# KTH-RPL/HiMo

Hardware: AMD Instinct MI355X
Metric: lidar_frames_per_sec_120k (higher is better)
Workload: dtype f16x2 (two-term split fp16, x = h + l with exact subnormals, on the matrix cores; float32 accumulate; ~22-bit products); 1 GPU; per-frame pipeline: pillarise 3 sweeps (512x512 grid) -> SeFlow++-style encoder/decoder + GRU head (random-init, self-specified: reference network source absent) -> per-point flow -> ego-motion removal + dt0 + flow2compDis -> comp_dis; points_per_frame=120000, sweeps_per_frame=3, parallelism=frames sharded x1, refined_output=False, batches_in_flight=3, matrix_arithmetic=f16x2, samples_per_backbone_launch=16, collectives=none (single process)

## Files before the change

### himo_amd/csrc/conv_common.h

```cpp
#pragma once
#include "himo_common.h"
#include "bf16x3.h"
#include <math.h>

namespace himo {

typedef float floatx16 __attribute__((ext_vector_type(16)));

enum Epilogue {
    kEpiBias = 0,
    kEpiBiasBnGelu = 1,
    kEpiBiasGelu = 2,
    kEpiGruZR = 3,
    kEpiGruQ = 4,
    kEpiBiasRelu = 5,
    kEpiReluMask = 6
};

struct ConvArgs {
    const float* x; int64_t x_batch_stride; int x_pitch;
    const float* w;
    const float* bias; const float* scale; const float* shift;
    float* y; int64_t y_batch_stride; int y_pitch;
    int N, H, W, Cin, Cout;
    int n_inner; int64_t x_outer_stride, y_outer_stride;
    int Ho, Wo;
    const float* aux_in; int aux_in_pitch;
    float* aux_out; int aux_out_pitch;
    int act_flags;
    unsigned* range_seen;
    const unsigned long long* mask;
    int64_t mask_batch_stride, mask_outer_stride;
};
enum ActFlags { kActSplitIn = 1, kActSplitOut = 2, kActVecStore = 4, kActAccumulate = 8, kActStuffedIn = 16, kActRowMask = 32 };

__device__ inline int64_t image_offset(int img, int n_inner, int64_t batch_stride, int64_t outer_stride) {
    return (int64_t)(img % n_inner) * batch_stride + (int64_t)(img / n_inner) * outer_stride;
}

__device__ inline int xcd_block_id(int bid, int n_blocks) {
    const int per = n_blocks >> 3, rem = n_blocks & 7;
    const int xcd = bid & 7, idx = bid >> 3;
    return xcd * per + (xcd < rem ? xcd : rem) + idx;
}

__device__ inline float gelu_exact(float v) {
    const float hv = 0.5f * v;
    const float t = __builtin_amdgcn_rcpf(fmaf(0.3275911f * 0.70710678118654752440f, fabsf(v), 1.0f));
    float p = fmaf(1.061405429f, t, -1.453152027f);
// ... 154 lines not shown
```

### himo_amd/csrc/conv_plan.h

```cpp
#pragma once
#include "conv_common.h"

namespace himo {

enum ConvFamily {
    kConvF32,
    kConvStaged,
    kConvFromL2,
    kConvPresplit3,
    kConvPresplit1
};

struct ConvPlan {
    ConvFamily family;
    ConvArgs args;
    int ks, stride, epi, fmt;
    int bn, mi, ph, nt;
    const void* w_packed;
    dim3 grid;
    const char* prof_name;
};

void launch_conv_f32(const ConvPlan& p, hipStream_t s);
void launch_conv_staged(const ConvPlan& p, hipStream_t s);
// ... 115 lines not shown
    a.H = d.h; a.W = d.w_in; a.Cin = d.cin; a.Cout = d.cout;
    a.Ho = d.stride == 2 ? (d.h + 1) / 2 : d.h;
    a.Wo = d.stride == 2 ? (d.w_in + 1) / 2 : d.w_in;
    a.aux_in = d.aux_in; a.aux_in_pitch = d.aux_in_pitch; a.aux_out = d.aux_out; a.aux_out_pitch = d.aux_out_pitch;
    a.act_flags = d.act_layout;
    a.range_seen = (d.act_layout & kActSplitOut) ? d.d_range_seen : nullptr;

    if (d.act_layout & kActRowMask) {
        if (!d.d_mask || (reinterpret_cast<uintptr_t>(d.d_mask) & 7u)) return HIMO_ERR_INVALID_ARGUMENT;
        if (d.act_layout != (kActRowMask | kActSplitIn) || !d.w_packed || d.packed_format != 1 || d.ksize != 3 || d.stride != 1 ||
            d.cout > 64 || (d.w_in & 31) || (d.epilogue != kEpiBias && d.epilogue != kEpiBiasBnGelu) || (d.cin & 15) || (d.x_pitch & 15))
            return HIMO_ERR_UNSUPPORTED;
        a.mask = reinterpret_cast<const unsigned long long*>(d.d_mask);
        a.mask_batch_stride = d.mask_batch_stride; a.mask_outer_stride = d.mask_outer_stride;
    }
    const bool gemm_acc = d.act_layout == kActAccumulate && d.w_packed && d.ksize == 1 && d.epilogue == kEpiBias && (d.packed_format == 0 || d.packed_format == 2);
    if (d.act_layout & (kActAccumulate | kActStuffedIn)) {
        if (!gemm_acc && ((d.act_layout & ~(kActAccumulate | kActStuffedIn)) || !d.w_packed || d.packed_format != 2 || d.ksize != 3 ||
                          d.stride != 1 || d.epilogue != kEpiBias))
            return HIMO_ERR_UNSUPPORTED;
        if ((d.act_layout & kActStuffedIn) && ((d.h & 1) || (d.w_in & 1) || !below_2gb((int64_t)(d.h / 2) * (d.w_in / 2), d.x_pitch)))
            return HIMO_ERR_UNSUPPORTED;
    } else if (d.act_layout && !(d.act_layout & kActRowMask)) {
        if ((d.act_layout & ~(kActSplitIn | kActSplitOut)) || !d.w_packed || d.packed_format != 1) return HIMO_ERR_UNSUPPORTED;
        if (d.ksize == 1 && !(d.act_layout & kActSplitIn)) return HIMO_ERR_UNSUPPORTED;
        if (d.epilogue != kEpiBias && d.epilogue != kEpiBiasBnGelu) return HIMO_ERR_UNSUPPORTED;
        if (((d.act_layout & kActSplitIn) && ((d.cin & 15) || (d.x_pitch & 15))) ||
            ((d.act_layout & kActSplitOut) && ((d.cout & 15) || (d.y_pitch & 15))))
            return HIMO_ERR_UNSUPPORTED;
    }

    const int hint = d.tile_hint, rows_hint = hint & 15;
    const bool l2_hint = hint == 0 || (hint & 0x1000);
    if (!d.w_packed || (d.stride == 2 && (gru || !l2_hint))) {
        p.family = kConvF32;
        plan_staged_tile(p, 4, 16, d.epilogue == kEpiGruZR, hint);
        p.prof_name = conv_prof_name(d.ksize, d.stride, -1);
        if (d.ksize == 1 && vec_store_ok(a) && !(a.Cout & 31) && (d.epilogue != kEpiReluMask || (aligned16(a.aux_in) && !(a.aux_in_pitch & 3))))
            a.act_flags |= kActVecStore;
// ... 20 lines not shown
```

### himo_amd/csrc/convsg.hip

```cpp
#include "conv_plan.h"
#include "bf16x3.h"
#include <type_traits>

namespace himo {

__device__ __attribute__((aligned(64))) unsigned char g_zero_page[64];


__device__ inline void glds16(const void* gsrc, unsigned lds_dst) {
    unsigned keep;
    asm volatile("s_mov_b32 %0, m0\n\ts_mov_b32 m0, %2\n\ts_nop 0\n\tglobal_load_lds_dwordx4 %1, off\n\ts_mov_b32 m0, %0"
                 : "=&s"(keep) : "v"(gsrc), "s"(lds_dst) : "memory");
}

template <int EPI, int PH, int MI, bool OSPLIT, int S, int NT = 1>
__global__ __launch_bounds__(256, NT == 2 ? (MI == 2 ? 3 : 2) : (S == 2 || MI == 4) ? 3 : 4)
void conv3_presplit_kernel(ConvArgs a, const unsigned short* __restrict__ wpk) {
    constexpr int TW = 32, TH = MI * PH, PHt = S == 1 ? TH + 2 : 2 * TH + 1, PWP = S == 1 ? 40 : 80, UPR = PWP / 16;
    constexpr int kRow = PWP * 64, kBuf = (PHt * kRow + 1023) / 1024 * 1024;
    constexpr int kUnits = S == 1 ? (PHt * PWP + 15) / 16 : PHt * UPR, kUPW = (kUnits + 3) / 4;
    constexpr int BN = (4 / PH) * 32 * NT;
    __shared__ __attribute__((aligned(1024))) unsigned char patch[2 * kBuf];

    const int n_tiles_n = (a.Cout + BN - 1) / BN;
    int bid = xcd_block_id(blockIdx.x, gridDim.x);
    const int tn = bid % n_tiles_n; bid /= n_tiles_n;
    const int tx = (a.Wo + TW - 1) / TW, ty = (a.Ho + TH - 1) / TH;
    const int ox0 = (bid % tx) * TW; bid /= tx;
    const int oy0 = (bid % ty) * TH;
    const int img = bid / ty;
    const unsigned char* __restrict__ xin = reinterpret_cast<const unsigned char*>(a.x + image_offset(img, a.n_inner, a.x_batch_stride, a.x_outer_stride));
    const int slabs = a.Cin >> 4;

    const int wave = __builtin_amdgcn_readfirstlane(threadIdx.x >> 6), lane = threadIdx.x & 63;
    const int wp = wave % PH, wc = wave / PH;
    const int li = lane & 31, lh = lane >> 5;
    const int co = tn * BN + wc * NT * 32 + li;
    const bool co_ok = co < a.Cout;
    const int iy0 = oy0 * S - 1, ix0 = ox0 * S - 1;
    const unsigned lds_base = (unsigned)(uintptr_t)(__attribute__((address_space(3))) unsigned char*)(&patch[0]);

    int src[kUPW];
#pragma unroll
    for (int k = 0; k < kUPW; ++k) {
        const int u = wave + 4 * k;
        const int q = u * 16 + (lane >> 2);
        const int row = S == 1 ? q / PWP : u / UPR, px = S == 1 ? q - row * PWP : (u % UPR) * 16 + (lane >> 2);
        const int col = S == 1 ? px : px < 48 ? 2 * px : 2 * (px - 48) + 1;
        const int iy = iy0 + row, ix = ix0 + col;
        const bool ok = u < kUnits && row < PHt && (S == 1 ? px < TW + 2 : px <= 32 || px >= 48) && iy >= 0 && iy < a.H && ix >= 0 && ix < a.W;
        const int sl = (lane & 3) ^ ((px >> 2) & 3);
        src[k] = ok ? (int)((((int64_t)iy * a.W + ix) * a.x_pitch) * 4 + sl * 16) : -1;
    }
    const unsigned char* zero = g_zero_page + (lane & 3) * 16;
    auto stage = [&](int slab, int buf) {
#pragma unroll
        for (int k = 0; k < kUPW; ++k) {
            const int u = wave + 4 * k;
            if (u < kUnits)
                glds16(src[k] >= 0 ? xin + (unsigned)(src[k] + slab * 64) : zero,
                       lds_base + buf * kBuf + (S == 1 ? u * 1024 : ((u / UPR) * PWP + (u % UPR) * 16) * 64));
        }
    };

    floatx16 acc[MI][NT];
#pragma unroll
    for (int mi = 0; mi < MI; ++mi)
#pragma unroll
        for (int nt = 0; nt < NT; ++nt)
#pragma unroll
            for (int r = 0; r < 16; ++r) acc[mi][nt][r] = 0.f;

    const unsigned char* __restrict__ wb = reinterpret_cast<const unsigned char*>(wpk);
    unsigned b_lane[NT];
#pragma unroll
    for (int nt = 0; nt < NT; ++nt) {
// ... 295 lines not shown
#pragma unroll
                for (int j = 0; j < 4; ++j) {
                    const int pxl = (four >> (8 * j)) & 255;
                    if (e0 + 8 * g + j < n_occ && co < a.Cout)
                        yout[((int64_t)(oy0 + (pxl >> 5)) * a.Wo + (ox0 + (pxl & 31))) * a.y_pitch + co] = epi_activate<EPI>(acc[mi][4 * g + j], eA, eB);
                }
            }
        }
    };
    if (mine_n == 1) { run(std::integral_constant<int, 1>{}); return; }
    if (mine_n == 2) { run(std::integral_constant<int, 2>{}); return; }
    if (mine_n == 3) { run(std::integral_constant<int, 3>{}); return; }
    run(std::integral_constant<int, 4>{});
}

template <int EPI, int PH, int MI, bool OSPLIT>
__global__ __launch_bounds__(256, 4)
void conv1_presplit_kernel(ConvArgs a, const unsigned short* __restrict__ wpk) {
    constexpr int G = 2, TH = MI * PH, BM = TH * 32;
    constexpr int kSeg = 32 * 64, kSlab = TH * kSeg, kBuf = G * kSlab;
    constexpr int kUnits = G * TH * 2, kUPW = (kUnits + 3) / 4;
    constexpr int BN = (4 / PH) * 32;
    __shared__ __attribute__((aligned(1024))) unsigned char patch[2 * kBuf < 16384 ? 16384 : 2 * kBuf];

    const int n_tiles_n = (a.Cout + BN - 1) / BN;
    int bid = xcd_block_id(blockIdx.x, gridDim.x);
    const int tn = bid % n_tiles_n; bid /= n_tiles_n;
    const int64_t rows = (int64_t)a.Ho * a.Wo;
    const int tiles = (int)((rows + BM - 1) / BM);
    const int img = bid / tiles;
    const int64_t row0 = (int64_t)(bid % tiles) * BM;
// ... 4 lines not shown
    const int wp = wave % PH, wc = wave / PH;
    const int li = lane & 31, lh = lane >> 5;
    const int co = tn * BN + wc * 32 + li;
    const bool co_ok = co < a.Cout;
    const unsigned lds_base = (unsigned)(uintptr_t)(__attribute__((address_space(3))) unsigned char*)(&patch[0]);

    int src[kUPW];
#pragma unroll
    for (int k = 0; k < kUPW; ++k) {
        const int u = wave + 4 * k;
        const int g = u / (2 * TH), seg = (u >> 1) % TH, px = (u & 1) * 16 + (lane >> 2);
        const int64_t pix = row0 + seg * 32 + px;
        const int sl = (lane & 3) ^ ((px >> 2) & 3);
        src[k] = (u < kUnits && pix < rows) ? (int)(pix * a.x_pitch * 4 + sl * 16 + g * 64) : -1;
    }
    const unsigned char* zero = g_zero_page + (lane & 3) * 16;
    auto stage = [&](int step, int buf) {
#pragma unroll
        for (int k = 0; k < kUPW; ++k) {
            const int u = wave + 4 * k;
            if (u < kUnits) {
                const int g = u / (2 * TH);
                const bool ok = src[k] >= 0 && step * G + g < slabs;
                glds16(ok ? xin + (unsigned)(src[k] + step * (G * 64)) : zero, lds_base + buf * kBuf + g * kSlab + ((u >> 1) % TH) * kSeg + (u & 1) * 1024);
            }
        }
    };

    floatx16 acc[MI];
#pragma unroll
    for (int mi = 0; mi < MI; ++mi)
#pragma unroll
        for (int r = 0; r < 16; ++r) acc[mi][r] = 0.f;

    const int co_ld = co_ok ? co : a.Cout - 1;
    const unsigned char* __restrict__ wb = reinterpret_cast<const unsigned char*>(wpk);
    const unsigned b_lane = (unsigned)co_ld * 32u + (unsigned)lh * 16u, b_plane = (unsigned)a.Cout * 32u;
    auto load_b = [&](int slab, uint4 (&b)[2]) {
        const unsigned off = (unsigned)slab * (2u * b_plane) + b_lane;
        b[0] = *reinterpret_cast<const uint4*>(wb + off);
// ... 70 lines not shown
                else yout[pix * a.y_pitch + co] = v;
            }
        }
    }
}

#define HIMO_SG(KERNEL, E, O, ...) hipLaunchKernelGGL((KERNEL<E, PH, MI, O, ##__VA_ARGS__>), p.grid, dim3(256), 0, s, p.args, (const unsigned short*)p.w_packed)
#define HIMO_SG_EPI(KERNEL, ...)                                                                                                          \
    do {                                                                                                                                  \
        const bool osplit = (p.args.act_flags & kActSplitOut) != 0;                                                                       \
        if (p.epi == kEpiBias) { if (osplit) HIMO_SG(KERNEL, kEpiBias, true, ##__VA_ARGS__); else HIMO_SG(KERNEL, kEpiBias, false, ##__VA_ARGS__); } \
        else { if (osplit) HIMO_SG(KERNEL, kEpiBiasBnGelu, true, ##__VA_ARGS__); else HIMO_SG(KERNEL, kEpiBiasBnGelu, false, ##__VA_ARGS__); }       \
    } while (0)

template <int PH, int MI>
static void launch_sg1(const ConvPlan& p, hipStream_t s) { HIMO_SG_EPI(conv1_presplit_kernel); }

template <int PH, int MI, int S = 1, int NT = 1>
static void launch_sg(const ConvPlan& p, hipStream_t s) { HIMO_SG_EPI(conv3_presplit_kernel, S, NT); }
#undef HIMO_SG_EPI
#undef HIMO_SG

void launch_conv_presplit1(const ConvPlan& p, hipStream_t s) {
    if (p.ph == 1) {
        if (p.mi == 4) launch_sg1<1, 4>(p, s);
        else if (p.mi == 2) launch_sg1<1, 2>(p, s);
        else launch_sg1<1, 1>(p, s);
    } else {
        if (p.mi == 2) launch_sg1<2, 2>(p, s);
        else launch_sg1<2, 1>(p, s);
    }
}

void launch_conv_presplit3(const ConvPlan& p, hipStream_t s) {
    if (p.args.act_flags & kActRowMask) {
        if (p.epi == kEpiBias) hipLaunchKernelGGL((conv3_rowmask_kernel<kEpiBias>), p.grid, dim3(256), 0, s, p.args, (const unsigned short*)p.w_packed);
        else hipLaunchKernelGGL((conv3_rowmask_kernel<kEpiBiasBnGelu>), p.grid, dim3(256), 0, s, p.args, (const unsigned short*)p.w_packed);
        return;
    }
    if (p.stride == 2) { if (p.ph == 1) launch_sg<1, 2, 2>(p, s); else launch_sg<2, 1, 2>(p, s); }
    else if (p.nt == 2) {
        if (p.ph == 4) launch_sg<4, 2, 1, 2>(p, s);
        else if (p.ph == 1) launch_sg<1, 4, 1, 2>(p, s);
        else launch_sg<2, 4, 1, 2>(p, s);
    }
    else if (p.ph == 1) {
        if (p.mi == 4) launch_sg<1, 4>(p, s);
        else if (p.mi == 2) launch_sg<1, 2>(p, s);
        else launch_sg<1, 1>(p, s);
    } else {
        if (p.mi == 2) launch_sg<2, 2>(p, s);
        else launch_sg<2, 1>(p, s);
    }
}

// ... 2 lines not shown
```

### himo_amd/pipeline.py

```python
from __future__ import annotations

from dataclasses import dataclass

import numpy as np
import torch

from . import _lib
from .compdis import CompDisEngine, FrameBatch
from .seflow.model import SeFlowNet


@dataclass
class Sample:
    pch1: torch.Tensor
    pc0: torch.Tensor
    pc1: torch.Tensor
    pose_h1: np.ndarray
    pose0: np.ndarray
    pose1: np.ndarray
    lidar_dt: torch.Tensor
    scene_id: str = ""
    timestamp: int = 0

    @classmethod
# ... 66 lines not shown
            meta=[(s.scene_id, s.timestamp) for s in samples])
        return self._batch

    def _forward(self, samples, outs) -> None:
        mb = self.net.max_batch
        for lo in range(0, len(samples), mb):
            grp = samples[lo:lo + mb]
            self.net.forward_batch([(s.pch1, s.pc0, s.pc1, s.pose_h1, s.pose0, s.pose1) for s in grp], outs[lo:lo + mb])

    def _set_sparse_dec4(self):
        net = self.net
        if hasattr(net, "sparse_dec4"):
            net.sparse_dec4 = bool(net.precision == "f16x2" and net.fused_head and net.split_acts)
            if hasattr(net, "head_offsets_only"):
                net.head_offsets_only = net.sparse_dec4

    def _fall_back(self):
        self.net = SeFlowNet(precision="bf16x3", **self._net_args)
        self._set_sparse_dec4()

    def _guard_begin(self):
        if self.net.precision == "f16x2":
            if not self.net.fused_head:
                raise RuntimeError("precision='f16x2' needs the fused head: its output stage carries the finite-flow guard")
            self.net.clear_nonfinite()

    def _guard_now(self) -> bool:
        if self.net.precision != "f16x2":
            return True
        self._guard_why = self.net.guard_verdict(self.net.guard.cpu().tolist())
# ... 150 lines not shown
```

### himo_amd/seflow/model.py

```python
from __future__ import annotations

import ctypes

import numpy as np
import torch

from .. import _lib
from . import spec

EPI_BIAS, EPI_BIAS_BN_GELU, EPI_BIAS_GELU, EPI_GRU_ZR, EPI_GRU_Q = range(5)


class ConvDesc(ctypes.Structure):
    _fields_ = [("x", ctypes.c_void_p), ("x_batch_stride", ctypes.c_int64), ("x_pitch", ctypes.c_int),
                ("w", ctypes.c_void_p), ("bias", ctypes.c_void_p), ("scale", ctypes.c_void_p), ("shift", ctypes.c_void_p),
                ("y", ctypes.c_void_p), ("y_batch_stride", ctypes.c_int64), ("y_pitch", ctypes.c_int),
                ("n", ctypes.c_int), ("h", ctypes.c_int), ("w_in", ctypes.c_int), ("cin", ctypes.c_int),
                ("cout", ctypes.c_int), ("ksize", ctypes.c_int), ("stride", ctypes.c_int), ("epilogue", ctypes.c_int),
                ("aux_in", ctypes.c_void_p), ("aux_in_pitch", ctypes.c_int),
                ("aux_out", ctypes.c_void_p), ("aux_out_pitch", ctypes.c_int), ("w_packed", ctypes.c_void_p),
                ("tile_hint", ctypes.c_int), ("packed_format", ctypes.c_int),
                ("n_outer", ctypes.c_int), ("x_outer_stride", ctypes.c_int64), ("y_outer_stride", ctypes.c_int64),
                ("act_layout", ctypes.c_int), ("range_seen", ctypes.c_void_p),
                ("mask", ctypes.c_void_p), ("mask_batch_stride", ctypes.c_int64), ("mask_outer_stride", ctypes.c_int64)]


ACT_SPLIT_IN, ACT_SPLIT_OUT = 1, 2
ACT_ROW_MASK = 32
ACT_ACCUMULATE = 8
ACT_STUFFED_2X = 16
PILLAR_NO_LISTS, PILLAR_HALFWAVE_ONLY = 4, 8


_lib.register({
    "himo_pillar_workspace_bytes": (ctypes.c_size_t, [ctypes.c_int64, ctypes.c_int, ctypes.c_int]),
    "himo_pillar_occupancy_reset": (ctypes.c_int, [ctypes.c_void_p, ctypes.c_size_t, ctypes.c_int, ctypes.c_int, ctypes.c_void_p]),
    "himo_pillarize": (ctypes.c_int, [ctypes.c_int64, ctypes.c_void_p, ctypes.c_int, ctypes.POINTER(ctypes.c_float),
                                      ctypes.POINTER(ctypes.c_float), ctypes.POINTER(ctypes.c_float),
                                      ctypes.POINTER(ctypes.c_float), ctypes.c_int, ctypes.c_int,
                                      ctypes.c_void_p, ctypes.c_void_p, ctypes.c_void_p,
                                      ctypes.c_void_p, ctypes.c_void_p, ctypes.c_void_p, ctypes.c_void_p,
                                      ctypes.c_int, ctypes.c_void_p, ctypes.c_size_t, ctypes.c_void_p]),
    "himo_conv2d": (ctypes.c_int, [ctypes.POINTER(ConvDesc), ctypes.c_void_p]),
# ... 92 lines not shown
            raise ValueError("max_batch")
        self.max_batch = max_batch
        self.precision = precision
        self.autotune = autotune
        self.keep_cell_lists = False
        self.fused_head = precision != "f32"
        self._incremental_images = True
        self.use_plan = True
        self.use_graph = True
        self._plans = {}
        self._recording = None
        self._nb = 1
        self.packed_format = 1 if precision == "f16x2" else 0
        self._split_acts = precision == "f16x2"
        self._sparse_dec4 = False
        self.head_offsets_only = False
        self.tiles = {}
        self.lib = _lib.load()
        self.device = device if device is not None else _lib.require_gpu()
        params = spec.init_params(seed) if params is None else params
        shapes = spec.param_shapes()
        for k, shp in shapes.items():
            if k not in params or tuple(params[k].shape) != tuple(shp):
                raise KeyError(f"parameter {k} missing or of wrong shape (want {shp})")
        cpu = {k: torch.from_numpy(np.ascontiguousarray(params[k], dtype=np.float32)) for k in shapes}
        def fold(prefix, eps):
            scale = cpu[f"{prefix}.gamma"] / torch.sqrt(cpu[f"{prefix}.var"] + eps)
            return scale, cpu[f"{prefix}.beta"] - cpu[f"{prefix}.mean"] * scale
        derived = {}
        derived["pfn.scale"], derived["pfn.shift"] = fold("pfn.bn", spec.BN_EPS_PFN)
# ... 45 lines not shown
        self.F1 = buf((H // 2) * (W // 2), 64 * F)
        self.E2 = [buf(F, (H // 4) * (W // 4), 128) for _ in range(2)]
        self.F2 = buf((H // 4) * (W // 4), 128 * F)
        self.E3 = [buf(F, (H // 8) * (W // 8), 256) for _ in range(2)]
        self.F3 = buf((H // 8) * (W // 8), 256 * F)
        self.T1 = buf((H // 8) * (W // 8), 256)
        self.CAT1 = buf((H // 4) * (W // 4), 512)
        self.S = [buf((H // 4) * (W // 4), 256) for _ in range(2)]
        self.T2 = buf((H // 4) * (W // 4), 128)
        self.CAT2 = buf((H // 2) * (W // 2), 256)
        self.T = [buf((H // 2) * (W // 2), 128) for _ in range(2)]
        self.T3 = buf((H // 2) * (W // 2), 64)
        self.CAT3 = buf(H * W, 128)
        self.U = [buf(H * W, 64) for _ in range(2)]
        self.DEC = buf(H * W, 64)
        self.occ0 = torch.zeros((B, (H * W + 63) // 64), dtype=torch.int64, device=dev)
        self.max_points = 0
        self._reserve_points(max_points)
        self.guard = torch.zeros(2 + self.MAX_RANGE_SLOTS, dtype=torch.int32, device=dev)
        self.nonfinite = self.guard[:1]
        self._ran_word = self.guard[-1:]
        self._range_slots = {}
        self._range = _f32x(spec.POINT_CLOUD_RANGE[:3])
        self._voxel = _f32x(spec.VOXEL_SIZE)
        r, v = spec.POINT_CLOUD_RANGE, spec.VOXEL_SIZE
        self._centre = _f32x([v[0] / 2 + r[0], v[1] / 2 + r[1], v[2] / 2 + r[2]])

    def _reserve_points(self, n: int):
        if n <= self.max_points:
            return
        dev = self.device
# ... 23 lines not shown
        if on != self._incremental_images:
            self._incremental_images = on
            self.reset_images()

    @property
    def split_acts(self) -> bool:
        return self._split_acts

    @split_acts.setter
    def split_acts(self, on: bool):
        on = bool(on)
        if on != self._split_acts:
            self._split_acts = on
            if not on:
                self._sparse_dec4 = False
            self.drop_plan()
            self.reset_images()

    HEAD_SLOT = 1

    @property
    def sparse_dec4(self) -> bool:
        return self._sparse_dec4

    @sparse_dec4.setter
    def sparse_dec4(self, on: bool):
        on = bool(on)
        if on and not (self.packed_format == 1 and self._split_acts and self.fused_head):
            raise ValueError("sparse_dec4 needs precision='f16x2' with split activations and the fused head")
        if on != self._sparse_dec4:
            self._sparse_dec4 = on
            self.drop_plan()

    @property
    def B0(self):
        return self._B0

    @B0.setter
    def B0(self, buf):
        self._B0 = buf
        self.drop_plan()
        self.reset_images()

    MAX_RANGE_SLOTS = 63

    def clear_nonfinite(self):
        _lib.check(self.lib.himo_clear_u32(self.guard.data_ptr(), self.guard.numel(), _lib.stream_handle()), "himo_clear_u32")

    def _range_word(self, wname: str) -> int:
# ... 11 lines not shown
        return None

    def reset_images(self):
        for st in getattr(self, "_pt", ()):
            for ws in st["ws_slots"]:
                _lib.check(self.lib.himo_pillar_occupancy_reset(ws.data_ptr(), ws.numel(), self.W, self.H, _lib.stream_handle()),
                           "himo_pillar_occupancy_reset")

    def _use_sample(self, i: int):
        st = self._pt[i]
        self._sample = i
        self.ws_slots, self.xyz_t, self.pid, self.offsets = st["ws_slots"], st["xyz_t"], st["pid"], st["offsets"]

    def _conv(self, x, x_bs, x_pitch, wname, y, y_bs, y_pitch, n, h, w, cin, cout, ks, stride, epi, x_off=0, y_off=0,
              scale=None, shift=None, aux_in=None, aux_in_pitch=0, aux_out=None, aux_out_pitch=0, bias=None, batched=True,
              act=0, mask=None):
        d = ConvDesc()
        d.x = x.data_ptr() + 4 * x_off; d.x_batch_stride = x_bs; d.x_pitch = x_pitch
        if batched and self._nb > 1:
            d.n_outer, d.x_outer_stride, d.y_outer_stride = self._nb, x.stride(0), y.stride(0)
        d.w = self.p[f"{wname}.weight"].data_ptr()
        d.bias = (self.p[f"{wname}.bias"] if bias is None else bias).data_ptr()
        d.scale = None if scale is None else scale.data_ptr()
        d.shift = None if shift is None else shift.data_ptr()
        d.y = y.data_ptr() + 4 * y_off; d.y_batch_stride = y_bs; d.y_pitch = y_pitch
        d.n, d.h, d.w_in, d.cin, d.cout, d.ksize, d.stride, d.epilogue = n, h, w, cin, cout, ks, stride, epi
        d.aux_in = None if aux_in is None else aux_in.data_ptr(); d.aux_in_pitch = aux_in_pitch
        d.aux_out = None if aux_out is None else aux_out.data_ptr(); d.aux_out_pitch = aux_out_pitch
        pk = self.packed.get(f"{wname}.weight")
        d.w_packed = None if pk is None else pk.data_ptr()
        d.packed_format = self.packed_format
        d.act_layout = act if self.split_acts else 0
        if mask is not None:
            d.act_layout |= ACT_ROW_MASK
            d.mask, d.mask_batch_stride, d.mask_outer_stride = mask.data_ptr(), 0, mask.stride(0)
        if (d.act_layout & ACT_SPLIT_OUT) and self.packed_format == 1 and epi in (EPI_BIAS, EPI_BIAS_BN_GELU):
            d.range_seen = self._range_word(wname)
        key = (n * max(d.n_outer, 1), h, w, cin, cout, ks, stride, epi, pk is not None, d.act_layout)
        if self.autotune and key not in self.tiles:
            self.tiles[key] = self._tune(d)
        d.tile_hint = self.tiles.get(key, 0)
        if self._recording is not None and epi not in (EPI_GRU_ZR, EPI_GRU_Q):
            op = HimoOp(); op.kind = 0; op.conv = d
            self._recording.append(op)
        _lib.check(self.lib.himo_conv2d(ctypes.byref(d), _lib.stream_handle()), f"himo_conv2d({wname})")

    def _tune(self, d: "ConvDesc") -> int:
        if d.epilogue in (EPI_GRU_ZR, EPI_GRU_Q) or (d.act_layout & ACT_ROW_MASK):
            return 0
        cands = [(bn << 4) | mi for bn in (128, 64) if not (bn == 128 and d.cout % 128) for mi in (2, 1)]
# ... 54 lines not shown
    def encoder(self):
        H, W, F = self.H, self.W, self.F
        p = self.p
        stages = [("enc1", 4, 32, 64, H, W, self.E1, self.F1), ("enc2", 6, 64, 128, H // 2, W // 2, self.E2, self.F2),
                  ("enc3", 6, 128, 256, H // 4, W // 4, self.E3, self.F3)]
        src, src_bs, src_pitch = self.B0, 32, 32 * F
        for stage, n_conv, cin, cout, h, w, pingpong, catbuf in stages:
            ho, wo = h // 2, w // 2
            for i in range(n_conv):
                name = f"{stage}.{i}"
                last = i == n_conv - 1
                dst = catbuf if last else pingpong[i % 2]
                dst_bs, dst_pitch = (cout, cout * F) if last else (ho * wo * cout, cout)
                act = ACT_SPLIT_IN | ACT_SPLIT_OUT
                if i == 0:
                    self._conv(src, src_bs, src_pitch, name, dst, dst_bs, dst_pitch, F, h, w, cin, cout, 3, 2,
                               EPI_BIAS_BN_GELU, scale=p[f"{name}.scale"], shift=p[f"{name}.shift"], act=act)
                else:
                    self._conv(src, src_bs, src_pitch, name, dst, dst_bs, dst_pitch, F, ho, wo, cout, cout, 3, 1,
                               EPI_BIAS_BN_GELU, scale=p[f"{name}.scale"], shift=p[f"{name}.shift"], act=act)
                src, src_bs, src_pitch = dst, dst_bs, dst_pitch

    def decoder(self):
        H, W, F = self.H, self.W, self.F
        IN, IO = ACT_SPLIT_IN, ACT_SPLIT_IN | ACT_SPLIT_OUT
        fold = self.fold_decoder
        def block(name, coarse, c_in, ch, cw, tmp, cat, skip, skip_c, lat, out, work, nxt=None):
            if coarse is not None:
                self._conv(coarse, 0, c_in, f"{name}.u1", tmp, 0, lat, 1, 1, ch * cw, c_in, lat, 1, 1, EPI_BIAS, act=IN)
            self._up(tmp, lat, ch, cw, lat, cat, 2 * lat, out_split=True)
            self._conv(skip, 0, skip_c, f"{name}.u3", cat, 0, 2 * lat, 1, 1, 4 * ch * cw, skip_c, lat, 1, 1, EPI_BIAS, y_off=lat, act=IO)
            self._conv(cat, 0, 2 * lat, f"{name}.u4", work[0], 0, out, 1, 2 * ch, 2 * cw, 2 * lat, out, 3, 1, EPI_BIAS, act=IO)
            if fold and nxt is not None:
                nname, ntmp, nlat = nxt
                self._conv(work[0], 0, out, f"{name}.u5>{nname}.u1", ntmp, 0, nlat, 1, 2 * ch, 2 * cw, out, nlat, 3, 1, EPI_BIAS, act=IN)
                return None
            self._conv(work[0], 0, out, f"{name}.u5", work[1], 0, out, 1, 2 * ch, 2 * cw, out, out, 3, 1, EPI_BIAS, act=IO)
            return work[1]
        s = block("dec1", self.F3, 256 * F, H // 8, W // 8, self.T1, self.CAT1, self.F2, 128 * F, 256, 256, self.S, ("dec2", self.T2, 128))
        t = block("dec2", s, 256, H // 4, W // 4, self.T2, self.CAT2, self.F1, 64 * F, 128, 128, self.T, ("dec3", self.T3, 64))
        u = block("dec3", t, 128, H // 2, W // 2, self.T3, self.CAT3, self.B0, 32 * F, 64, 64, self.U)
        self._conv(u, 0, 64, "dec4", self.DEC, 0, 64, 1, H, W, 64, 64, 3, 1, EPI_BIAS, act=IN,
                   mask=self.occ0 if self._sparse_dec4 else None)
        return self.DEC

    def head(self, pc0: torch.Tensor, slot0: int = 1, slot1: int = 2, out: torch.Tensor | None = None) -> torch.Tensor:
# ... 112 lines not shown
        lean = self.head_offsets_only and not self.keep_cell_lists
        for lo in range(0, len(jobs), per_call):
            grp = jobs[lo:lo + per_call]
            arr = (HimoSweep * (len(grp) * self.F))()
            for j, (sample, sweeps, transforms) in enumerate(grp):
                st = self._pt[sample]
                for slot, (pts, T) in enumerate(zip(sweeps, transforms)):
                    w = arr[j * self.F + slot]
                    w.n, w.d_pts, w.pc_stride = pts.shape[0], pts.data_ptr(), pts.shape[1]
                    w.transform = _f32x(np.asarray(T, dtype=np.float32).reshape(-1))
                    w.d_xyz_t, w.d_pid, w.d_offsets = st["xyz_t"][slot].data_ptr(), st["pid"][slot].data_ptr(), st["offsets"][slot].data_ptr()
                    if lean and slot != self.HEAD_SLOT:
                        w.d_offsets = None
                    w.d_image = self.B0[sample].data_ptr() + 4 * 32 * slot
                    w.d_workspace = st["ws_slots"][slot].data_ptr()
                    w.d_occupancy = self.occ0[sample].data_ptr() if slot == self.HEAD_SLOT else None
            status = self.lib.himo_pillarize_multi_ex(len(arr), ctypes.addressof(arr), self._range, self._voxel, self._centre, self.W, self.H,
                                                      self.p["pfn.weight"].data_ptr(), self.p["pfn.scale"].data_ptr(),
                                                      self.p["pfn.shift"].data_ptr(), 32 * self.F, self._pt[0]["ws_slots"][0].numel(),
                                                      (1 if self.split_acts else 0) | (2 if self.incremental_images else 0) |
                                                      (PILLAR_NO_LISTS if lean else 0), _lib.stream_handle())
            _lib.check(status, "himo_pillarize_multi_ex")

    def pillar_features(self, sweeps, transforms, scale: torch.Tensor, shift: torch.Tensor):
        arr = (HimoSweep * self.F)()
        st = self._pt[self._sample]
        for slot, (pts, T) in enumerate(zip(sweeps, transforms)):
            w = arr[slot]
            w.n, w.d_pts, w.pc_stride = pts.shape[0], pts.data_ptr(), pts.shape[1]
            w.transform = _f32x(np.asarray(T, dtype=np.float32).reshape(-1))
            w.d_xyz_t, w.d_pid, w.d_offsets = st["xyz_t"][slot].data_ptr(), st["pid"][slot].data_ptr(), st["offsets"][slot].data_ptr()
# ... 3 lines not shown
                                                     self.p["pfn.weight"].data_ptr(), scale.data_ptr(), shift.data_ptr(), 32 * self.F,
                                                     st["ws_slots"][0].numel(),
                                                     (1 if self.split_acts else 0) | (2 if self.incremental_images else 0), _lib.stream_handle())
        _lib.check(status, "himo_pillar_features_multi")

    def pillarize_into(self, slot: int, pts: torch.Tensor, transform):
        n = pts.shape[0]
        self._reserve_points(n)
        arr = (HimoSweep * 1)()
        w = arr[0]
        w.n, w.d_pts, w.pc_stride = n, pts.data_ptr(), pts.shape[1]
        w.transform = _f32x(np.asarray(transform, dtype=np.float32).reshape(-1))
        w.d_xyz_t, w.d_pid, w.d_offsets = self.xyz_t[slot].data_ptr(), self.pid[slot].data_ptr(), self.offsets[slot].data_ptr()
        w.d_image = self.B0[self._sample].data_ptr() + 4 * 32 * slot
        w.d_workspace = self.ws_slots[slot].data_ptr()
        w.d_occupancy = self.occ0[self._sample].data_ptr() if slot == self.HEAD_SLOT else None
        st = self.lib.himo_pillarize_multi_ex(1, ctypes.addressof(arr), self._range, self._voxel, self._centre, self.W, self.H,
                                              self.p["pfn.weight"].data_ptr(), self.p["pfn.scale"].data_ptr(),
                                              self.p["pfn.shift"].data_ptr(), 32 * self.F, self.ws_slots[slot].numel(),
                                              (1 if self.split_acts else 0) | (2 if self.incremental_images else 0), _lib.stream_handle())
        _lib.check(st, "himo_pillarize_multi_ex")


def conv2d_nhwc(x: torch.Tensor, weight: torch.Tensor, bias: torch.Tensor, stride: int = 1, epilogue: int = EPI_BIAS,
                scale: torch.Tensor | None = None, shift: torch.Tensor | None = None, precision: str = "f32",
                tile_hint: int = 0, act_layout: int = 0, out: torch.Tensor | None = None) -> torch.Tensor:
    lib = _lib.load()
    n, h, w, cin = x.shape
    k, _, _, cout = weight.shape
    stuffed = bool(act_layout & ACT_STUFFED_2X)
    if stuffed:
# ... 32 lines not shown
```

### include/himo_amd.h

```cpp
#ifndef HIMO_AMD_H
#define HIMO_AMD_H

#include <stddef.h>
#include <stdint.h>

#ifdef __cplusplus
extern "C" {
#endif

#define HIMO_ABI_VERSION 1

typedef enum himo_status {
    HIMO_OK = 0,
    HIMO_ERR_INVALID_ARGUMENT = 1,
    HIMO_ERR_EMPTY_FRAME = 2,
    HIMO_ERR_WORKSPACE = 3,
    HIMO_ERR_SINGULAR_POSE = 4,
    HIMO_ERR_HIP = 5,
    HIMO_ERR_UNSUPPORTED = 6
} himo_status;

#define HIMO_FLAG_F32_CHAIN 0x1u
#define HIMO_FLAG_RAW 0x2u
#define HIMO_FLAG_SCANIA 0x4u
// ... 397 lines not shown
    const float* w;
    const float* bias; const float* scale; const float* shift;
    float* y; int64_t y_batch_stride; int y_pitch;
    int n, h, w_in, cin, cout, ksize, stride, epilogue;
    const float* aux_in; int aux_in_pitch;
    float* aux_out; int aux_out_pitch;
    const void* w_packed;
    int tile_hint;
    int packed_format;
    int n_outer;
    int64_t x_outer_stride, y_outer_stride;
    int act_layout;
    uint32_t* d_range_seen;
    const uint64_t* d_mask;
    int64_t mask_batch_stride, mask_outer_stride;
} himo_conv_desc;
#define HIMO_ACT_SPLIT_IN 1
#define HIMO_ACT_SPLIT_OUT 2
#define HIMO_ACT_ROW_MASK 32
#define HIMO_ACT_ACCUMULATE 8
#define HIMO_ACT_STUFFED_2X 16
int himo_conv2d(const himo_conv_desc* h_desc, void* stream);
size_t himo_conv_packed_weight_bytes(int ksize, int cin, int cout);
int himo_conv_pack_weights(const float* d_w, int ksize, int cin, int cout, void* d_packed, void* stream);
#define HIMO_PACK_BF16X3 0
#define HIMO_PACK_F16X2 1
#define HIMO_PACK_BF16X2 2
int himo_conv_pack_weights_ex(const float* d_w, int ksize, int cin, int cout, int format, void* d_packed, void* stream);

int himo_upsample2x(const float* d_x, int x_pitch, int h, int w, int c, float* d_y, int y_pitch, void* stream);
int himo_upsample2x_batch(int n, const float* d_x, int64_t x_batch_stride, int x_pitch, int h, int w, int c, float* d_y,
                          int64_t y_batch_stride, int y_pitch, void* stream);
int himo_upsample2x_batch_ex(int n, const float* d_x, int64_t x_batch_stride, int x_pitch, int h, int w, int c, float* d_y,
                             int64_t y_batch_stride, int y_pitch, int out_split, void* stream);
// ... 279 lines not shown
```

Baseline: 772.6 frames/s.

## Skip loading empty pillars in first encoder and skip convs via occupancy masks

The pillarize step now writes a per-sweep occupancy bitmask for all slots instead of only the head slot. The first stride-2 encoder conv and the decoder's 1x1 skip conv on B0 read these masks and stage zeros from a zero page for unoccupied pixels, per channel group, instead of fetching them from global memory. This cuts global memory traffic on the sparse pillar image. The cost is extra mask reads and bit bookkeeping in the staging loops, plus more template variants.

```diff
diff --git a/himo_amd/csrc/conv_common.h b/himo_amd/csrc/conv_common.h
--- a/himo_amd/csrc/conv_common.h
+++ b/himo_amd/csrc/conv_common.h
@@ -31,8 +31,9 @@
     unsigned* range_seen;
     const unsigned long long* mask;
     int64_t mask_batch_stride, mask_outer_stride;
+    int mask_group_steps; int64_t mask_group_stride;
 };
-enum ActFlags { kActSplitIn = 1, kActSplitOut = 2, kActVecStore = 4, kActAccumulate = 8, kActStuffedIn = 16, kActRowMask = 32 };
+enum ActFlags { kActSplitIn = 1, kActSplitOut = 2, kActVecStore = 4, kActAccumulate = 8, kActStuffedIn = 16, kActRowMask = 32, kActInMask = 64 };
 
 __device__ inline int64_t image_offset(int img, int n_inner, int64_t batch_stride, int64_t outer_stride) {
     return (int64_t)(img % n_inner) * batch_stride + (int64_t)(img / n_inner) * outer_stride;
diff --git a/himo_amd/csrc/conv_plan.h b/himo_amd/csrc/conv_plan.h
--- a/himo_amd/csrc/conv_plan.h
+++ b/himo_amd/csrc/conv_plan.h
@@ -153,6 +153,17 @@
         a.mask = reinterpret_cast<const unsigned long long*>(d.d_mask);
         a.mask_batch_stride = d.mask_batch_stride; a.mask_outer_stride = d.mask_outer_stride;
     }
+    if (d.act_layout & kActInMask) {
+        if (!d.d_mask || (reinterpret_cast<uintptr_t>(d.d_mask) & 7u) || d.mask_group_channels < 0) return HIMO_ERR_INVALID_ARGUMENT;
+        const int gch = d.mask_group_channels ? d.mask_group_channels : d.cin;
+        if ((d.act_layout & ~(kActInMask | kActSplitIn | kActSplitOut)) || !(d.act_layout & kActSplitIn) || !d.w_packed || d.packed_format != 1 ||
+            !(d.ksize == 1 || d.stride == 2) || (d.ksize == 3 && d.tile_hint && !(d.tile_hint & 0x1000)) ||
+            (gch & 31) || d.cin % gch || d.cin / gch > 32)
+            return HIMO_ERR_UNSUPPORTED;
+        a.mask = reinterpret_cast<const unsigned long long*>(d.d_mask);
+        a.mask_batch_stride = d.mask_batch_stride; a.mask_outer_stride = d.mask_outer_stride;
+        a.mask_group_steps = gch / (d.ksize == 1 ? 32 : 16); a.mask_group_stride = d.mask_group_stride;
+    }
     const bool gemm_acc = d.act_layout == kActAccumulate && d.w_packed && d.ksize == 1 && d.epilogue == kEpiBias && (d.packed_format == 0 || d.packed_format == 2);
     if (d.act_layout & (kActAccumulate | kActStuffedIn)) {
         if (!gemm_acc && ((d.act_layout & ~(kActAccumulate | kActStuffedIn)) || !d.w_packed || d.packed_format != 2 || d.ksize != 3 ||
@@ -161,7 +172,7 @@
         if ((d.act_layout & kActStuffedIn) && ((d.h & 1) || (d.w_in & 1) || !below_2gb((int64_t)(d.h / 2) * (d.w_in / 2), d.x_pitch)))
             return HIMO_ERR_UNSUPPORTED;
     } else if (d.act_layout && !(d.act_layout & kActRowMask)) {
-        if ((d.act_layout & ~(kActSplitIn | kActSplitOut)) || !d.w_packed || d.packed_format != 1) return HIMO_ERR_UNSUPPORTED;
+        if ((d.act_layout & ~(kActSplitIn | kActSplitOut | kActInMask)) || !d.w_packed || d.packed_format != 1) return HIMO_ERR_UNSUPPORTED;
         if (d.ksize == 1 && !(d.act_layout & kActSplitIn)) return HIMO_ERR_UNSUPPORTED;
         if (d.epilogue != kEpiBias && d.epilogue != kEpiBiasBnGelu) return HIMO_ERR_UNSUPPORTED;
         if (((d.act_layout & kActSplitIn) && ((d.cin & 15) || (d.x_pitch & 15))) ||
diff --git a/himo_amd/csrc/convsg.hip b/himo_amd/csrc/convsg.hip
--- a/himo_amd/csrc/convsg.hip
+++ b/himo_amd/csrc/convsg.hip
@@ -13,7 +13,7 @@
                  : "=&s"(keep) : "v"(gsrc), "s"(lds_dst) : "memory");
 }
 
-template <int EPI, int PH, int MI, bool OSPLIT, int S, int NT = 1>
+template <int EPI, int PH, int MI, bool OSPLIT, int S, int NT = 1, bool IM = false>
 __global__ __launch_bounds__(256, NT == 2 ? (MI == 2 ? 3 : 2) : (S == 2 || MI == 4) ? 3 : 4)
 void conv3_presplit_kernel(ConvArgs a, const unsigned short* __restrict__ wpk) {
     constexpr int TW = 32, TH = MI * PH, PHt = S == 1 ? TH + 2 : 2 * TH + 1, PWP = S == 1 ? 40 : 80, UPR = PWP / 16;
@@ -41,6 +41,10 @@
     const unsigned lds_base = (unsigned)(uintptr_t)(__attribute__((address_space(3))) unsigned char*)(&patch[0]);
 
     int src[kUPW];
+    unsigned occ[kUPW];
+    int grp_left = IM ? a.mask_group_steps : 0;
+    const unsigned* __restrict__ mw = IM ? reinterpret_cast<const unsigned*>(a.mask + image_offset(img, a.n_inner, a.mask_batch_stride, a.mask_outer_stride)) : nullptr;
+    const int groups = IM ? slabs / a.mask_group_steps : 0;
 #pragma unroll
     for (int k = 0; k < kUPW; ++k) {
         const int u = wave + 4 * k;
@@ -51,6 +55,14 @@
         const bool ok = u < kUnits && row < PHt && (S == 1 ? px < TW + 2 : px <= 32 || px >= 48) && iy >= 0 && iy < a.H && ix >= 0 && ix < a.W;
         const int sl = (lane & 3) ^ ((px >> 2) & 3);
         src[k] = ok ? (int)((((int64_t)iy * a.W + ix) * a.x_pitch) * 4 + sl * 16) : -1;
+        if (IM) {
+            occ[k] = 0u;
+            if (ok) {
+                const int pix = iy * a.W + ix;
+                for (int g = 0; g < groups; ++g)
+                    occ[k] |= ((mw[2 * (g * a.mask_group_stride) + (pix >> 5)] >> (pix & 31)) & 1u) << g;
+            }
+        }
     }
     const unsigned char* zero = g_zero_page + (lane & 3) * 16;
     auto stage = [&](int slab, int buf) {
@@ -58,8 +70,13 @@
         for (int k = 0; k < kUPW; ++k) {
             const int u = wave + 4 * k;
             if (u < kUnits)
-                glds16(src[k] >= 0 ? xin + (unsigned)(src[k] + slab * 64) : zero,
+                glds16((IM ? (occ[k] & 1u) != 0 : src[k] >= 0) ? xin + (unsigned)(src[k] + slab * 64) : zero,
                        lds_base + buf * kBuf + (S == 1 ? u * 1024 : ((u / UPR) * PWP + (u % UPR) * 16) * 64));
+        }
+        if (IM && --grp_left == 0) {
+            grp_left = a.mask_group_steps;
+#pragma unroll
+            for (int k = 0; k < kUPW; ++k) occ[k] >>= 1;
         }
     };
 
@@ -385,7 +402,7 @@
     run(std::integral_constant<int, 4>{});
 }
 
-template <int EPI, int PH, int MI, bool OSPLIT>
+template <int EPI, int PH, int MI, bool OSPLIT, bool IM = false>
 __global__ __launch_bounds__(256, 4)
 void conv1_presplit_kernel(ConvArgs a, const unsigned short* __restrict__ wpk) {
     constexpr int G = 2, TH = MI * PH, BM = TH * 32;
@@ -420,6 +437,28 @@
         const int sl = (lane & 3) ^ ((px >> 2) & 3);
         src[k] = (u < kUnits && pix < rows) ? (int)(pix * a.x_pitch * 4 + sl * 16 + g * 64) : -1;
     }
+    unsigned occ[kUPW];
+    int grp_left = IM ? a.mask_group_steps : 0;
+    if (IM) {
+        const unsigned long long* __restrict__ mw = a.mask + image_offset(img, a.n_inner, a.mask_batch_stride, a.mask_outer_stride);
+        const int groups = steps / a.mask_group_steps;
+#pragma unroll
+        for (int k = 0; k < kUPW; ++k) occ[k] = 0u;
+        for (int g = 0; g < groups; ++g) {
+#pragma unroll
+            for (int k = 0; k < kUPW; ++k) {
+                const int u = wave + 4 * k;
+                const int64_t pix0 = row0 + ((u >> 1) % TH) * 32 + (u & 1) * 16;
+                if (u < kUnits && pix0 < rows) {
+                    const unsigned long long word = mw[g * a.mask_group_stride + (pix0 >> 6)];
+                    occ[k] |= (unsigned)((word >> ((int)(pix0 & 63) + (lane >> 2))) & 1ull) << g;
+                }
+            }
+        }
+#pragma unroll
+        for (int k = 0; k < kUPW; ++k)
+            if (src[k] < 0) occ[k] = 0u;
+    }
     const unsigned char* zero = g_zero_page + (lane & 3) * 16;
     auto stage = [&](int step, int buf) {
 #pragma unroll
@@ -427,9 +466,14 @@
             const int u = wave + 4 * k;
             if (u < kUnits) {
                 const int g = u / (2 * TH);
-                const bool ok = src[k] >= 0 && step * G + g < slabs;
+                const bool ok = (IM ? (occ[k] & 1u) != 0 : src[k] >= 0) && step * G + g < slabs;
                 glds16(ok ? xin + (unsigned)(src[k] + step * (G * 64)) : zero, lds_base + buf * kBuf + g * kSlab + ((u >> 1) % TH) * kSeg + (u & 1) * 1024);
             }
+        }
+        if (IM && --grp_left == 0) {
+            grp_left = a.mask_group_steps;
+#pragma unroll
+            for (int k = 0; k < kUPW; ++k) occ[k] >>= 1;
         }
     };
 
@@ -530,10 +574,13 @@
     } while (0)
 
 template <int PH, int MI>
-static void launch_sg1(const ConvPlan& p, hipStream_t s) { HIMO_SG_EPI(conv1_presplit_kernel); }
-
-template <int PH, int MI, int S = 1, int NT = 1>
-static void launch_sg(const ConvPlan& p, hipStream_t s) { HIMO_SG_EPI(conv3_presplit_kernel, S, NT); }
+static void launch_sg1(const ConvPlan& p, hipStream_t s) {
+    if (p.args.act_flags & kActInMask) { HIMO_SG_EPI(conv1_presplit_kernel, true); }
+    else { HIMO_SG_EPI(conv1_presplit_kernel); }
+}
+
+template <int PH, int MI, int S = 1, int NT = 1, bool IM = false>
+static void launch_sg(const ConvPlan& p, hipStream_t s) { HIMO_SG_EPI(conv3_presplit_kernel, S, NT, IM); }
 #undef HIMO_SG_EPI
 #undef HIMO_SG
 
@@ -554,7 +601,8 @@
         else hipLaunchKernelGGL((conv3_rowmask_kernel<kEpiBiasBnGelu>), p.grid, dim3(256), 0, s, p.args, (const unsigned short*)p.w_packed);
         return;
     }
-    if (p.stride == 2) { if (p.ph == 1) launch_sg<1, 2, 2>(p, s); else launch_sg<2, 1, 2>(p, s); }
+    if (p.stride == 2 && (p.args.act_flags & kActInMask)) { if (p.ph == 1) launch_sg<1, 2, 2, 1, true>(p, s); else launch_sg<2, 1, 2, 1, true>(p, s); }
+    else if (p.stride == 2) { if (p.ph == 1) launch_sg<1, 2, 2>(p, s); else launch_sg<2, 1, 2>(p, s); }
     else if (p.nt == 2) {
         if (p.ph == 4) launch_sg<4, 2, 1, 2>(p, s);
         else if (p.ph == 1) launch_sg<1, 4, 1, 2>(p, s);
diff --git a/himo_amd/pipeline.py b/himo_amd/pipeline.py
--- a/himo_amd/pipeline.py
+++ b/himo_amd/pipeline.py
@@ -104,6 +104,8 @@
             net.sparse_dec4 = bool(net.precision == "f16x2" and net.fused_head and net.split_acts)
             if hasattr(net, "head_offsets_only"):
                 net.head_offsets_only = net.sparse_dec4
+        if hasattr(net, "input_occupancy"):
+            net.input_occupancy = bool(net.precision == "f16x2" and net.split_acts)
 
     def _fall_back(self):
         self.net = SeFlowNet(precision="bf16x3", **self._net_args)
diff --git a/himo_amd/seflow/model.py b/himo_amd/seflow/model.py
--- a/himo_amd/seflow/model.py
+++ b/himo_amd/seflow/model.py
@@ -22,11 +22,13 @@
                 ("tile_hint", ctypes.c_int), ("packed_format", ctypes.c_int),
                 ("n_outer", ctypes.c_int), ("x_outer_stride", ctypes.c_int64), ("y_outer_stride", ctypes.c_int64),
                 ("act_layout", ctypes.c_int), ("range_seen", ctypes.c_void_p),
-                ("mask", ctypes.c_void_p), ("mask_batch_stride", ctypes.c_int64), ("mask_outer_stride", ctypes.c_int64)]
+                ("mask", ctypes.c_void_p), ("mask_batch_stride", ctypes.c_int64), ("mask_outer_stride", ctypes.c_int64),
+                ("mask_group_channels", ctypes.c_int), ("mask_group_stride", ctypes.c_int64)]
 
 
 ACT_SPLIT_IN, ACT_SPLIT_OUT = 1, 2
 ACT_ROW_MASK = 32
+ACT_IN_MASK = 64
 ACT_ACCUMULATE = 8
 ACT_STUFFED_2X = 16
 PILLAR_NO_LISTS, PILLAR_HALFWAVE_ONLY = 4, 8
@@ -149,6 +151,7 @@
         self.packed_format = 1 if precision == "f16x2" else 0
         self._split_acts = precision == "f16x2"
         self._sparse_dec4 = False
+        self._input_occupancy = False
         self.head_offsets_only = False
         self.tiles = {}
         self.lib = _lib.load()
@@ -224,7 +227,8 @@
         self.CAT3 = buf(H * W, 128)
         self.U = [buf(H * W, 64) for _ in range(2)]
         self.DEC = buf(H * W, 64)
-        self.occ0 = torch.zeros((B, (H * W + 63) // 64), dtype=torch.int64, device=dev)
+        self.occ = torch.zeros((B, F, (H * W + 63) // 64), dtype=torch.int64, device=dev)
+        self.occ0 = self.occ[:, self.HEAD_SLOT]
         self.max_points = 0
         self._reserve_points(max_points)
         self.guard = torch.zeros(2 + self.MAX_RANGE_SLOTS, dtype=torch.int32, device=dev)
@@ -278,6 +282,7 @@
             self._split_acts = on
             if not on:
                 self._sparse_dec4 = False
+                self._input_occupancy = False
             self.drop_plan()
             self.reset_images()
 
@@ -297,6 +302,19 @@
             self.drop_plan()
 
     @property
+    def input_occupancy(self) -> bool:
+        return self._input_occupancy
+
+    @input_occupancy.setter
+    def input_occupancy(self, on: bool):
+        on = bool(on)
+        if on and not (self.packed_format == 1 and self._split_acts):
+            raise ValueError("input_occupancy needs precision='f16x2' with split activations")
+        if on != self._input_occupancy:
+            self._input_occupancy = on
+            self.drop_plan()
+
+    @property
     def B0(self):
         return self._B0
 
@@ -338,7 +356,7 @@
 
     def _conv(self, x, x_bs, x_pitch, wname, y, y_bs, y_pitch, n, h, w, cin, cout, ks, stride, epi, x_off=0, y_off=0,
               scale=None, shift=None, aux_in=None, aux_in_pitch=0, aux_out=None, aux_out_pitch=0, bias=None, batched=True,
-              act=0, mask=None):
+              act=0, mask=None, in_mask=None):
         d = ConvDesc()
         d.x = x.data_ptr() + 4 * x_off; d.x_batch_stride = x_bs; d.x_pitch = x_pitch
         if batched and self._nb > 1:
@@ -358,6 +376,11 @@
         if mask is not None:
             d.act_layout |= ACT_ROW_MASK
             d.mask, d.mask_batch_stride, d.mask_outer_stride = mask.data_ptr(), 0, mask.stride(0)
+        if in_mask is not None:
+            masks, mask_bs, group_ch = in_mask
+            d.act_layout |= ACT_IN_MASK
+            d.mask, d.mask_batch_stride, d.mask_outer_stride = masks.data_ptr(), mask_bs, masks.stride(0)
+            d.mask_group_channels, d.mask_group_stride = group_ch, masks.stride(1)
         if (d.act_layout & ACT_SPLIT_OUT) and self.packed_format == 1 and epi in (EPI_BIAS, EPI_BIAS_BN_GELU):
             d.range_seen = self._range_word(wname)
         key = (n * max(d.n_outer, 1), h, w, cin, cout, ks, stride, epi, pk is not None, d.act_layout)
@@ -442,8 +465,9 @@
                 dst_bs, dst_pitch = (cout, cout * F) if last else (ho * wo * cout, cout)
                 act = ACT_SPLIT_IN | ACT_SPLIT_OUT
                 if i == 0:
+                    occ = (self.occ, self.occ.stride(1), cin) if (self._input_occupancy and src is self.B0) else None
                     self._conv(src, src_bs, src_pitch, name, dst, dst_bs, dst_pitch, F, h, w, cin, cout, 3, 2,
-                               EPI_BIAS_BN_GELU, scale=p[f"{name}.scale"], shift=p[f"{name}.shift"], act=act)
+                               EPI_BIAS_BN_GELU, scale=p[f"{name}.scale"], shift=p[f"{name}.shift"], act=act, in_mask=occ)
                 else:
                     self._conv(src, src_bs, src_pitch, name, dst, dst_bs, dst_pitch, F, ho, wo, cout, cout, 3, 1,
                                EPI_BIAS_BN_GELU, scale=p[f"{name}.scale"], shift=p[f"{name}.shift"], act=act)
@@ -457,7 +481,9 @@
             if coarse is not None:
                 self._conv(coarse, 0, c_in, f"{name}.u1", tmp, 0, lat, 1, 1, ch * cw, c_in, lat, 1, 1, EPI_BIAS, act=IN)
             self._up(tmp, lat, ch, cw, lat, cat, 2 * lat, out_split=True)
-            self._conv(skip, 0, skip_c, f"{name}.u3", cat, 0, 2 * lat, 1, 1, 4 * ch * cw, skip_c, lat, 1, 1, EPI_BIAS, y_off=lat, act=IO)
+            occ = (self.occ, 0, 32) if (self._input_occupancy and skip is self.B0) else None
+            self._conv(skip, 0, skip_c, f"{name}.u3", cat, 0, 2 * lat, 1, 1, 4 * ch * cw, skip_c, lat, 1, 1, EPI_BIAS, y_off=lat, act=IO,
+                       in_mask=occ)
             self._conv(cat, 0, 2 * lat, f"{name}.u4", work[0], 0, out, 1, 2 * ch, 2 * cw, 2 * lat, out, 3, 1, EPI_BIAS, act=IO)
             if fold and nxt is not None:
                 nname, ntmp, nlat = nxt
@@ -600,7 +626,7 @@
                         w.d_offsets = None
                     w.d_image = self.B0[sample].data_ptr() + 4 * 32 * slot
                     w.d_workspace = st["ws_slots"][slot].data_ptr()
-                    w.d_occupancy = self.occ0[sample].data_ptr() if slot == self.HEAD_SLOT else None
+                    w.d_occupancy = self.occ[sample, slot].data_ptr()
             status = self.lib.himo_pillarize_multi_ex(len(arr), ctypes.addressof(arr), self._range, self._voxel, self._centre, self.W, self.H,
                                                       self.p["pfn.weight"].data_ptr(), self.p["pfn.scale"].data_ptr(),
                                                       self.p["pfn.shift"].data_ptr(), 32 * self.F, self._pt[0]["ws_slots"][0].numel(),
@@ -634,7 +660,7 @@
         w.d_xyz_t, w.d_pid, w.d_offsets = self.xyz_t[slot].data_ptr(), self.pid[slot].data_ptr(), self.offsets[slot].data_ptr()
         w.d_image = self.B0[self._sample].data_ptr() + 4 * 32 * slot
         w.d_workspace = self.ws_slots[slot].data_ptr()
-        w.d_occupancy = self.occ0[self._sample].data_ptr() if slot == self.HEAD_SLOT else None
+        w.d_occupancy = self.occ[self._sample, slot].data_ptr()
         st = self.lib.himo_pillarize_multi_ex(1, ctypes.addressof(arr), self._range, self._voxel, self._centre, self.W, self.H,
                                               self.p["pfn.weight"].data_ptr(), self.p["pfn.scale"].data_ptr(),
                                               self.p["pfn.shift"].data_ptr(), 32 * self.F, self.ws_slots[slot].numel(),
diff --git a/include/himo_amd.h b/include/himo_amd.h
--- a/include/himo_amd.h
+++ b/include/himo_amd.h
@@ -435,10 +435,13 @@
     uint32_t* d_range_seen;
     const uint64_t* d_mask;
     int64_t mask_batch_stride, mask_outer_stride;
+    int mask_group_channels;
+    int64_t mask_group_stride;
 } himo_conv_desc;
 #define HIMO_ACT_SPLIT_IN 1
 #define HIMO_ACT_SPLIT_OUT 2
 #define HIMO_ACT_ROW_MASK 32
+#define HIMO_ACT_IN_MASK 64
 #define HIMO_ACT_ACCUMULATE 8
 #define HIMO_ACT_STUFFED_2X 16
 int himo_conv2d(const himo_conv_desc* h_desc, void* stream);
```

Measured after the change: 775.7 frames/s, median of 6. Within noise of the previous version (+0.4%).
